# fxxJuses/MICFormer

Hardware: AMD Instinct MI355X
Metric: train volumes/sec (128^3 CT+MRI pair) (higher is better)
Workload: dtype bf16; 1 GPU; MicFormer base Head(embed_dim=48, depths 2-2-6-2, heads 3-6-12-24, window 2^3, 8 classes) full train step (fwd + MDiceLoss + bwd + Adam/cosine) on 128^3 CT+MR pairs, DropPath on; local_batch=2, global_batch=2, parallelism=dp1, launch=hipGraph replay (one graph)

## Files before the change

### micformer_amd/csrc/common.h

```cpp
#pragma once
#include <hip/hip_runtime.h>
#include <stdint.h>

#include "../../include/micformer_hip.h"
#include "gemm_core.h"

#define MICF_RETURN_LAUNCH()                          \
  do {                                                \
    return hipGetLastError() == hipSuccess ? MICF_OK : MICF_ELAUNCH; \
  } while (0)

namespace micf {

struct Options {
  int block_wave = 1;
  int block_recompute_h = 0;
  int block_debug = 0;
  int sample_tile = 1;
  int sample_e = -1;
  int cell_cap = -1;
  int tile_cap_hits = -1, tile_cap_cell = -1, tile_cap_voxel = -1;
};
Options& options();

struct Geo {
  int B, D, H, W;
  FastDiv fW, fH, fD;
  Geo() {}
  Geo(int B_, int D_, int H_, int W_) : B(B_), D(D_), H(H_), W(W_), fW((uint32_t)W_), fH((uint32_t)H_), fD((uint32_t)D_) {}
  __host__ __device__ int64_t tokens() const { return (int64_t)B * D * H * W; }
  __device__ __forceinline__ void decode(int t, int& b, int& d, int& h, int& w) const {
    uint32_t q, r;
    fW.divmod((uint32_t)t, q, r); w = (int)r;
    fH.divmod(q, q, r); h = (int)r;
    fD.divmod(q, q, r); d = (int)r; b = (int)q;
  }
  __device__ __forceinline__ int token(int b, int d, int h, int w) const { return ((b * D + d) * H + h) * W + w; }
};

__device__ __forceinline__ float wave_sum(float v) {
#pragma unroll
  for (int o = 32; o > 0; o >>= 1) v += __shfl_xor(v, o, 64);
  return v;
}

int colsum_atomic(const float* dy, const float* scale, int64_t rps, float* out, int64_t M, int N, hipStream_t s);

constexpr int kOffsetHidden = 16;
struct CellLists {
  int* count;
  int* ovf_count;
  int* list;
  int* ovf;
  int cap;
  float* w8;
};
struct SampleFwdSet { const float *h, *ln_g, *ln_b, *w1, *xa; float *flow, *xs; };
struct SampleBwdSet {
  const float *dxs, *h, *ln_g, *ln_b, *w1, *xa, *flow;
  float *dxa, *dh, *dln_g, *dln_b, *dw1;
  CellLists cl;
  float* partials;
};
int offset_sample_fwd_groups(const SampleFwdSet* sets, int n, int B, int D, int H, int W, int C, float eps, hipStream_t stream);
int offset_sample_bwd_groups(SampleBwdSet* sets, int n, int B, int D, int H, int W, int C, float eps, float* workspace,
                             int64_t workspace_floats, hipStream_t s, int phase = 0);
struct SampleFinishCall { const SampleBwdSet* sets; int n, B, D, H, W, C; float* workspace; int64_t workspace_floats; };
int offset_sample_finish_many(const SampleFinishCall* calls, int ncalls, hipStream_t s);

struct Conv3FwdSet { const float* x1; const float* x2; const float* w; const float* bias; float* y; float* wt; };
struct Conv3BwdSet { const float* dy; const float* w; float* wt; float* dx1; float* dx2; };
int conv3_fwd_x_groups(const Conv3FwdSet* sets, int n, int c1, int c2, int B, int D, int H, int W, int N, hipStream_t stream, int dtype,
                       int prepared, int y_zeroed);
bool conv3_fwd_x_splits(int B, int D, int H, int W, int c1, int c2);
int conv3_bwd_data_x_groups(const Conv3BwdSet* sets, int ng, int c1, int acc1, int c2, int acc2, int B, int D, int H, int W, int N,
                            hipStream_t stream, int dtype, int prepared);

int conv3_bwd_data_x(const float* dy, const float* w, float* wt, float* dx1, int c1, int acc1, float* dx2, int c2, int acc2, int B,
                     int D, int H, int W, int N, hipStream_t stream, int dtype = 0, int prepared = 0);

int64_t conv3_fwdx_workspace(int N, int c1, int c2);
int conv3_fwd_x(const float* x1, int c1, const float* x2, int c2, const float* w, const float* bias, float* y, float* wt, int B, int D,
                int H, int W, int N, hipStream_t stream, int dtype = 0, int prepared = 0);
int64_t conv3_wgradx_workspace(int B, int D, int H, int W, int N, int c1, int c2, int items = 1);
int conv3_wgradx_items(const float* const* dy, const float* const* x1, const float* const* x2, float* const* dw, float* const* dbias,
                       int n, int c1, int c2, int B, int D, int H, int W, int N, float* ws, int64_t ws_floats, hipStream_t stream,
                       int dtype);
int conv3_wgradx(const float* dy, const float* x1, int c1, const float* x2, int c2, float* dw, float* dbias, int B, int D, int H,
                 int W, int N, float* ws, int64_t ws_floats, hipStream_t stream, int dtype = 0);

}
```

### micformer_amd/csrc/conv3_bwdx.hip

```cpp
#include <cstdlib>
#include "common.h"
#include "conv3_layout.h"
#include "gemm_dma.h"

namespace micf {

constexpr int xKS = 20;

struct BwdxArgs {
  const float* dy; int N;
  const float* wt;
  float* d1; float* d2; int oc1, oc2, acc1, acc2;
  int O;
  int B, D, H, W, tiles_d, tiles_h, tiles_w, ngroups;
  const float* dyb; const float* wtb; float* d1b; float* d2b;
};

__global__ void __launch_bounds__(256) conv3_wt_kernel(const float* __restrict__ w, float* __restrict__ wt, int N, int Cin) {
  const int64_t id = (int64_t)blockIdx.x * 256 + threadIdx.x;
  if (id < conv3_bwd_layout_items(Cin)) conv3_bwd_layout_write(w, wt, N, Cin, id);
}

template <int TW, int NCT, bool BF16>
__global__ void __launch_bounds__(256) conv3_bwdx_kernel(BwdxArgs a) {
  constexpr int CH = 16 / TW, TH = 4 * CH, TD = 2;
  constexpr int HD = TD + 2, HH = TH + 2, HW = TW + 2, HALO = HD * HH * HW;
  __shared__ __attribute__((aligned(16))) float Xs[HALO * xKS];
  if (blockIdx.z) { a.dy = a.dyb; a.wt = a.wtb; a.d1 = a.d1b; a.d2 = a.d2b; }
  const int tid = threadIdx.x, lane = tid & 63, wave = __builtin_amdgcn_readfirstlane(tid >> 6), li = lane & 15, lr = lane >> 4;
  int q = blockIdx.x;
  if (gridDim.x >= 64 && (gridDim.x & 7) == 0) q = (q & 7) * (gridDim.x >> 3) + (q >> 3);
  const int tw = q % a.tiles_w; q /= a.tiles_w;
  const int th = q % a.tiles_h; q /= a.tiles_h;
  const int td = q % a.tiles_d; const int b = q / a.tiles_d;
  const int d0 = td * TD, h0 = th * TH, w0 = tw * TW;
  const int64_t DHW = (int64_t)a.D * a.H * a.W;
  const int ct0 = blockIdx.y * NCT;
  const int nct = min(NCT, a.O / 16 - ct0);

  {
    constexpr int NH = (HALO * 4 + 255) / 256;
    float4 hv4[NH];
#pragma unroll
    for (int it = 0; it < NH; ++it) {
      const int idx = tid + it * 256;
      hv4[it] = make_float4(0.f, 0.f, 0.f, 0.f);
      if (idx < HALO * 4) {
        const int hv = idx >> 2, g = idx & 3;
        const int hw = hv % HW, hh = (hv / HW) % HH, hd = hv / (HW * HH);
        const int dd = d0 + hd - 1, yy = h0 + hh - 1, ww = w0 + hw - 1;
        if ((unsigned)dd < (unsigned)a.D && (unsigned)yy < (unsigned)a.H && (unsigned)ww < (unsigned)a.W && 4 * g < a.N)
          hv4[it] = *reinterpret_cast<const float4*>(a.dy + ((int64_t)b * DHW + ((int64_t)dd * a.H + yy) * a.W + ww) * a.N + 4 * g);
      }
    }
#pragma unroll
    for (int it = 0; it < NH; ++it) {
      const int idx = tid + it * 256;
      if (idx < HALO * 4) {
        if constexpr (BF16)
          *reinterpret_cast<uint2*>(&reinterpret_cast<uint16_t*>(Xs)[(idx >> 2) * xKS + 4 * (idx & 3)]) =
              make_uint2(pack_bf16(hv4[it].x, hv4[it].y), pack_bf16(hv4[it].z, hv4[it].w));
        else
          *reinterpret_cast<float4*>(&Xs[(idx >> 2) * xKS + 4 * (idx & 3)]) = hv4[it];
      }
    }
  }
  int ld[2], lh[2], lw[2];
#pragma unroll
  for (int tj = 0; tj < 2; ++tj) {
    const int ct = 2 * wave + tj;
    ld[tj] = ct / 4;
    lh[tj] = (ct % 4) * CH + li / TW;
    lw[tj] = li % TW;
  }
  f32x4 acc[NCT][2];
#pragma unroll
  for (int t = 0; t < NCT; ++t) { acc[t][0] = f32x4{0.f, 0.f, 0.f, 0.f}; acc[t][1] = f32x4{0.f, 0.f, 0.f, 0.f}; }
  const float* wp = a.wt + ((int64_t)(ct0 * 16 + li)) * 16 + 4 * lr;
  const int64_t tap_stride = (int64_t)a.O * 16;
  if constexpr (BF16) {
    typedef unsigned u32x4 __attribute__((ext_vector_type(4)));
    const uint16_t* Xh = reinterpret_cast<const uint16_t*>(Xs);
    const u32x4* wq = reinterpret_cast<const u32x4*>(reinterpret_cast<const uint16_t*>(a.wt + conv3_bwd_layout_f32(a.O)) +
                                                     (((int64_t)(ct0 * 16 + li)) * 4 + lr) * 8);
    const int64_t pair_stride = (int64_t)a.O * 4;
// ... 64 lines not shown
  for (int t = 0; t < NCT; ++t) av[t] = (t < nct && !BF16) ? *reinterpret_cast<const float4*>(wp + t * 256) : make_float4(0.f, 0.f, 0.f, 0.f);
  if constexpr (!BF16) __syncthreads();
#pragma unroll 1
  for (int tap = 0; tap < (BF16 ? 0 : 27); ++tap) {
    if (tap + 1 < 27) {
#pragma unroll
      for (int t = 0; t < NCT; ++t)
        an[t] = (t < nct) ? *reinterpret_cast<const float4*>(wp + (tap + 1) * tap_stride + t * 256) : make_float4(0.f, 0.f, 0.f, 0.f);
    }
    const int kd = tap / 9, kh = (tap / 3) % 3, kw = tap % 3;
    float4 bv[2];
#pragma unroll
    for (int tj = 0; tj < 2; ++tj) {
      const int zd = ld[tj] + 2 - kd, zh = lh[tj] + 2 - kh, zw = lw[tj] + 2 - kw;
      bv[tj] = *reinterpret_cast<const float4*>(&Xs[((zd * HH + zh) * HW + zw) * xKS + 4 * lr]);
    }
    if constexpr (!BF16) {
#pragma unroll
      for (int s = 0; s < 4; ++s) {
        const float b0 = s == 0 ? bv[0].x : (s == 1 ? bv[0].y : (s == 2 ? bv[0].z : bv[0].w));
        const float b1 = s == 0 ? bv[1].x : (s == 1 ? bv[1].y : (s == 2 ? bv[1].z : bv[1].w));
#pragma unroll
        for (int t = 0; t < NCT; ++t) {
          const float av_s = s == 0 ? av[t].x : (s == 1 ? av[t].y : (s == 2 ? av[t].z : av[t].w));
          acc[t][0] = __builtin_amdgcn_mfma_f32_16x16x4f32(av_s, b0, acc[t][0], 0, 0, 0);
          acc[t][1] = __builtin_amdgcn_mfma_f32_16x16x4f32(av_s, b1, acc[t][1], 0, 0, 0);
        }
      }
    } else {
      if ((tap & 1) || tap == 26) {
        const float4 z = make_float4(0.f, 0.f, 0.f, 0.f);
        const bool pair = tap & 1;
        const bf16x8 bb0 = pair ? to_bf16x8(bprev[0], bv[0]) : to_bf16x8(bv[0], z);
        const bf16x8 bb1 = pair ? to_bf16x8(bprev[1], bv[1]) : to_bf16x8(bv[1], z);
#pragma unroll
        for (int t = 0; t < NCT; ++t) {
          const bf16x8 ba = pair ? to_bf16x8(aprev[t], av[t]) : to_bf16x8(av[t], z);
          acc[t][0] = __builtin_amdgcn_mfma_f32_16x16x32_bf16(ba, bb0, acc[t][0], 0, 0, 0);
          acc[t][1] = __builtin_amdgcn_mfma_f32_16x16x32_bf16(ba, bb1, acc[t][1], 0, 0, 0);
        }
      } else {
        bprev[0] = bv[0]; bprev[1] = bv[1];
#pragma unroll
        for (int t = 0; t < NCT; ++t) aprev[t] = av[t];
      }
    }
#pragma unroll
    for (int t = 0; t < NCT; ++t) av[t] = an[t];
  }
#pragma unroll
  for (int tj = 0; tj < 2; ++tj) {
    const int dd = d0 + ld[tj], yy = h0 + lh[tj], ww = w0 + lw[tj];
    if (dd >= a.D || yy >= a.H || ww >= a.W) continue;
    const int64_t tok = (int64_t)b * DHW + ((int64_t)dd * a.H + yy) * a.W + ww;
    auto where = [&](int t, int& accf) -> float* {
      const int c = (ct0 + t) * 16 + 4 * lr;
      if (t >= nct) return nullptr;
      if (c < a.oc1) { accf = a.acc1; return a.d1 ? a.d1 + tok * a.oc1 + c : nullptr; }
      accf = a.acc2;
      return a.d2 ? a.d2 + tok * a.oc2 + (c - a.oc1) : nullptr;
    };
    constexpr int EB = NCT >= 6 ? 2 : NCT;
#pragma unroll
    for (int t0 = 0; t0 < NCT; t0 += EB) {
      float4 old[EB];
#pragma unroll
      for (int u = 0; u < EB; ++u) {
        int accf = 0;
        const float* p = where(t0 + u, accf);
        old[u] = (p && accf) ? *reinterpret_cast<const float4*>(p) : make_float4(0.f, 0.f, 0.f, 0.f);
      }
#pragma unroll
      for (int u = 0; u < EB; ++u) {
        int accf = 0;
        float* p = where(t0 + u, accf);
        if (!p) continue;
        const f32x4 v = acc[t0 + u][tj];
        *reinterpret_cast<float4*>(p) = make_float4(v[0] + old[u].x, v[1] + old[u].y, v[2] + old[u].z, v[3] + old[u].w);
      }
    }
  }
}

template <int TW, bool BF16>
static hipError_t launch_bwdx(BwdxArgs& a, hipStream_t stream) {
  constexpr int CH = 16 / TW, TH = 4 * CH;
  a.tiles_d = (a.D + 1) / 2;
  a.tiles_h = (a.H + TH - 1) / TH;
  a.tiles_w = (a.W + TW - 1) / TW;
  const int64_t blocks = (int64_t)a.B * a.tiles_d * a.tiles_h * a.tiles_w;
  const int cts = a.O / 16;
  if (blocks * ((cts + 5) / 6) >= 128)
    hipLaunchKernelGGL((conv3_bwdx_kernel<TW, 6, BF16>), dim3((unsigned)blocks, (cts + 5) / 6, a.ngroups), dim3(256), 0, stream, a);
  else
    hipLaunchKernelGGL((conv3_bwdx_kernel<TW, 2, BF16>), dim3((unsigned)blocks, (cts + 1) / 2, a.ngroups), dim3(256), 0, stream, a);
  return hipGetLastError();
}

int conv3_bwd_data_x(const float* dy, const float* w, float* wt, float* dx1, int c1, int acc1, float* dx2, int c2, int acc2, int B,
                     int D, int H, int W, int N, hipStream_t stream, int dtype, int prepared) {
  const Conv3BwdSet one{dy, w, wt, dx1, dx2};
  return conv3_bwd_data_x_groups(&one, 1, c1, acc1, c2, acc2, B, D, H, W, N, stream, dtype, prepared);
}

int conv3_bwd_data_x_groups(const Conv3BwdSet* sets, int ng, int c1, int acc1, int c2, int acc2, int B, int D, int H, int W, int N,
                            hipStream_t stream, int dtype, int prepared) {
  if (!sets || ng < 1 || ng > 2) return MICF_EINVAL;
  const int O = c1 + c2;
  if (N > 16 || (N & 3) || (O & 15) || (c1 & 3) || (c2 & 3) || W < 4) return MICF_EUNSUPPORTED;
  for (int i = 0; i < ng; ++i)
    if (!aligned16(sets[i].dy) || !aligned16(sets[i].wt) || (sets[i].dx1 && !aligned16(sets[i].dx1)) || (sets[i].dx2 && !aligned16(sets[i].dx2)) ||
        (!sets[i].dx1) != (!sets[0].dx1) || (!sets[i].dx2) != (!sets[0].dx2))
      return MICF_EUNSUPPORTED;
  const float *dy = sets[0].dy;
  float *wt = sets[0].wt, *dx1 = sets[0].dx1, *dx2 = sets[0].dx2;
  const int64_t n = conv3_bwd_layout_items(O);
  if (!prepared) {
    for (int i = 0; i < ng; ++i) {
      hipLaunchKernelGGL(conv3_wt_kernel, dim3((unsigned)((n + 255) / 256)), dim3(256), 0, stream, sets[i].w, sets[i].wt, N, O);
      if (hipGetLastError() != hipSuccess) return MICF_ELAUNCH;
    }
  }
  BwdxArgs a{};
  a.dyb = sets[ng - 1].dy; a.wtb = sets[ng - 1].wt; a.d1b = sets[ng - 1].dx1; a.d2b = sets[ng - 1].dx2; a.ngroups = ng;
  a.dy = dy; a.N = N; a.wt = wt; a.d1 = dx1; a.d2 = dx2; a.oc1 = c1; a.oc2 = c2; a.acc1 = acc1; a.acc2 = acc2; a.O = O;
  a.B = B; a.D = D; a.H = H; a.W = W;
  const hipError_t e = dtype == MICF_DTYPE_BF16 ? ((W >= 12) ? launch_bwdx<16, true>(a, stream) : launch_bwdx<8, true>(a, stream))
                                                 : ((W >= 12) ? launch_bwdx<16, false>(a, stream) : launch_bwdx<8, false>(a, stream));
  return e == hipSuccess ? MICF_OK : MICF_ELAUNCH;
}

}
```

### micformer_amd/csrc/conv3_fwdx.hip

```cpp
#include <cstdlib>
#include "common.h"
#include "conv3_layout.h"
#include "gemm_dma.h"

namespace micf {

constexpr int fKS = 20;
constexpr int fAhead = 3;

struct FwdxArgs {
  const float* x1; const float* x2; int c1, c2;
  const float* wt;
  const float* bias; float* y; int N;
  const float* x1b; const float* x2b; const float* wtb; const float* biasb; float* yb;
  int B, D, H, W, tiles_d, tiles_h, tiles_w;
  int chunks, chunks_per_block;
};

__global__ void __launch_bounds__(256) conv3_wtf_kernel(const float* __restrict__ w, float* __restrict__ wt, int N, int Cin, int chunks) {
  const int64_t id = (int64_t)blockIdx.x * 256 + threadIdx.x;
  if (id < conv3_fwd_layout_items(Cin)) conv3_fwd_layout_write(w, wt, N, Cin, id);
}

template <int TW, bool BF16>
__global__ void __launch_bounds__(256) conv3_fwdx_kernel(FwdxArgs a) {
  constexpr int CH = 16 / TW, TH = 4 * CH, TD = 2;
  constexpr int HD = TD + 2, HH = TH + 2, HW = TW + 2, HALO = HD * HH * HW;
  constexpr int NH = (HALO * 4 + 255) / 256;
  __shared__ __attribute__((aligned(16))) float Xs[HALO * fKS];
  if (blockIdx.z) { a.x1 = a.x1b; a.x2 = a.x2b; a.wt = a.wtb; a.bias = a.biasb; a.y = a.yb; }
  const int tid = threadIdx.x, lane = tid & 63, wave = __builtin_amdgcn_readfirstlane(tid >> 6), li = lane & 15, lr = lane >> 4;
  int q = blockIdx.x;
  if (gridDim.x >= 64 && (gridDim.x & 7) == 0) q = (q & 7) * (gridDim.x >> 3) + (q >> 3);
  const int tw = q % a.tiles_w; q /= a.tiles_w;
  const int th = q % a.tiles_h; q /= a.tiles_h;
  const int td = q % a.tiles_d; const int b = q / a.tiles_d;
  const int d0 = td * TD, h0 = th * TH, w0 = tw * TW;
  const int64_t DHW = (int64_t)a.D * a.H * a.W;
  const int Cin = a.c1 + a.c2;
  const int kc_begin = blockIdx.y * a.chunks_per_block;
  const int kc_end = min(a.chunks, kc_begin + a.chunks_per_block);

  auto fetch = [&](int kc, float4 (&hv)[NH]) {
#pragma unroll
    for (int it = 0; it < NH; ++it) {
      const int idx = tid + it * 256;
      hv[it] = make_float4(0.f, 0.f, 0.f, 0.f);
      if (idx < HALO * 4) {
        const int v = idx >> 2, g = idx & 3;
        const int hw = v % HW, hh = (v / HW) % HH, hd = v / (HW * HH);
        const int dd = d0 + hd - 1, yy = h0 + hh - 1, ww = w0 + hw - 1;
        const int c = kc * 16 + 4 * g;
        if ((unsigned)dd < (unsigned)a.D && (unsigned)yy < (unsigned)a.H && (unsigned)ww < (unsigned)a.W && c < Cin) {
          const int64_t tok = (int64_t)b * DHW + ((int64_t)dd * a.H + yy) * a.W + ww;
          hv[it] = c < a.c1 ? *reinterpret_cast<const float4*>(a.x1 + tok * a.c1 + c)
                            : *reinterpret_cast<const float4*>(a.x2 + tok * a.c2 + (c - a.c1));
        }
      }
    }
  };
  uint16_t* Xh = reinterpret_cast<uint16_t*>(Xs);
  auto commit = [&](const float4 (&hv)[NH]) {
#pragma unroll
    for (int it = 0; it < NH; ++it) {
      const int idx = tid + it * 256;
      if (idx < HALO * 4) {
        if constexpr (BF16)
          *reinterpret_cast<uint2*>(&Xh[(idx >> 2) * fKS + 4 * (idx & 3)]) = make_uint2(pack_bf16(hv[it].x, hv[it].y), pack_bf16(hv[it].z, hv[it].w));
        else
          *reinterpret_cast<float4*>(&Xs[(idx >> 2) * fKS + 4 * (idx & 3)]) = hv[it];
      }
    }
  };

  int vbase[2];
#pragma unroll
  for (int tj = 0; tj < 2; ++tj) {
    const int ct = 2 * wave + tj;
    const int ld = ct / 4, lh = (ct % 4) * CH + li / TW, lw = li % TW;
    vbase[tj] = ((ld * HH + lh) * HW + lw) * fKS + 4 * lr;
  }
  f32x4 acc[2] = {f32x4{0.f, 0.f, 0.f, 0.f}, f32x4{0.f, 0.f, 0.f, 0.f}};
  float4 hv[NH];
  fetch(kc_begin, hv);
  for (int kc = kc_begin; kc < kc_end; ++kc) {
// ... 17 lines not shown
#pragma unroll
        for (int e = 0; e < 2; ++e) {
          const int tap = 2 * p + e;
          if (tap < 27) {
            const int kd = tap / 9, kh = (tap / 3) % 3, kw = tap % 3;
            const int off = ((kd * HH + kh) * HW + kw) * fKS;
            h[e][0] = *reinterpret_cast<const uint2*>(&Xh[vbase[0] + off]);
            h[e][1] = *reinterpret_cast<const uint2*>(&Xh[vbase[1] + off]);
          } else {
            h[e][0] = make_uint2(0u, 0u); h[e][1] = h[e][0];
          }
        }
        const u32x4 q0 = {h[0][0].x, h[0][0].y, h[1][0].x, h[1][0].y}, q1 = {h[0][1].x, h[0][1].y, h[1][1].x, h[1][1].y};
        acc[0] = __builtin_amdgcn_mfma_f32_16x16x32_bf16(__builtin_bit_cast(bf16x8, aq), __builtin_bit_cast(bf16x8, q0), acc[0], 0, 0, 0);
        acc[1] = __builtin_amdgcn_mfma_f32_16x16x32_bf16(__builtin_bit_cast(bf16x8, aq), __builtin_bit_cast(bf16x8, q1), acc[1], 0, 0, 0);
      }
      continue;
    }
    float4 ring[fAhead + 1];
    float4 aprev = make_float4(0.f, 0.f, 0.f, 0.f);
    uint2 hprev0 = make_uint2(0u, 0u), hprev1 = hprev0;
#pragma unroll
    for (int t = 0; t < fAhead; ++t) ring[t] = *reinterpret_cast<const float4*>(wp + t * 256);
#pragma unroll
    for (int tap = 0; tap < 27; ++tap) {
      if (tap + fAhead < 27) ring[(tap + fAhead) % (fAhead + 1)] = *reinterpret_cast<const float4*>(wp + (tap + fAhead) * 256);
      const float4 av = ring[tap % (fAhead + 1)];
      const int kd = tap / 9, kh = (tap / 3) % 3, kw = tap % 3;
      const int off = ((kd * HH + kh) * HW + kw) * fKS;
      if constexpr (!BF16) {
        const float4 b0 = *reinterpret_cast<const float4*>(&Xs[vbase[0] + off]);
        const float4 b1 = *reinterpret_cast<const float4*>(&Xs[vbase[1] + off]);
        acc[0] = __builtin_amdgcn_mfma_f32_16x16x4f32(av.x, b0.x, acc[0], 0, 0, 0);
        acc[1] = __builtin_amdgcn_mfma_f32_16x16x4f32(av.x, b1.x, acc[1], 0, 0, 0);
        acc[0] = __builtin_amdgcn_mfma_f32_16x16x4f32(av.y, b0.y, acc[0], 0, 0, 0);
        acc[1] = __builtin_amdgcn_mfma_f32_16x16x4f32(av.y, b1.y, acc[1], 0, 0, 0);
        acc[0] = __builtin_amdgcn_mfma_f32_16x16x4f32(av.z, b0.z, acc[0], 0, 0, 0);
        acc[1] = __builtin_amdgcn_mfma_f32_16x16x4f32(av.z, b1.z, acc[1], 0, 0, 0);
        acc[0] = __builtin_amdgcn_mfma_f32_16x16x4f32(av.w, b0.w, acc[0], 0, 0, 0);
        acc[1] = __builtin_amdgcn_mfma_f32_16x16x4f32(av.w, b1.w, acc[1], 0, 0, 0);
      } else {
        typedef unsigned u32x4 __attribute__((ext_vector_type(4)));
        const uint2 h0 = *reinterpret_cast<const uint2*>(&Xh[vbase[0] + off]);
        const uint2 h1 = *reinterpret_cast<const uint2*>(&Xh[vbase[1] + off]);
        if ((tap & 1) || tap == 26) {
          const float4 z = make_float4(0.f, 0.f, 0.f, 0.f);
          const bool pair = tap & 1;
          const bf16x8 ba = pair ? to_bf16x8(aprev, av) : to_bf16x8(av, z);
          const u32x4 q0 = pair ? u32x4{hprev0.x, hprev0.y, h0.x, h0.y} : u32x4{h0.x, h0.y, 0u, 0u};
          const u32x4 q1 = pair ? u32x4{hprev1.x, hprev1.y, h1.x, h1.y} : u32x4{h1.x, h1.y, 0u, 0u};
          acc[0] = __builtin_amdgcn_mfma_f32_16x16x32_bf16(ba, __builtin_bit_cast(bf16x8, q0), acc[0], 0, 0, 0);
          acc[1] = __builtin_amdgcn_mfma_f32_16x16x32_bf16(ba, __builtin_bit_cast(bf16x8, q1), acc[1], 0, 0, 0);
        } else {
          aprev = av; hprev0 = h0; hprev1 = h1;
        }
      }
    }
  }
  const bool atomic_out = gridDim.y > 1;
  const int n0 = 4 * lr;
#pragma unroll
  for (int tj = 0; tj < 2; ++tj) {
    const int ct = 2 * wave + tj;
    const int dd = d0 + ct / 4, yy = h0 + (ct % 4) * CH + li / TW, ww = w0 + li % TW;
    if (dd >= a.D || yy >= a.H || ww >= a.W || n0 >= a.N) continue;
    float* p = a.y + ((int64_t)b * DHW + ((int64_t)dd * a.H + yy) * a.W + ww) * a.N + n0;
    f32x4 v = acc[tj];
    if (a.bias && blockIdx.y == 0) {
#pragma unroll
      for (int e = 0; e < 4; ++e) if (n0 + e < a.N) v[e] += a.bias[n0 + e];
    }
    if (atomic_out) {
#pragma unroll
      for (int e = 0; e < 4; ++e) if (n0 + e < a.N) atomicAdd(p + e, v[e]);
    } else if (n0 + 3 < a.N && (a.N & 3) == 0) {
      *reinterpret_cast<float4*>(p) = make_float4(v[0], v[1], v[2], v[3]);
    } else {
#pragma unroll
      for (int e = 0; e < 4; ++e) if (n0 + e < a.N) p[e] = v[e];
    }
  }
}

int64_t conv3_fwdx_workspace(int N, int c1, int c2) {
  if (N <= 0 || N > 16 || c1 + c2 <= 0) return 0;
  return conv3_fwd_layout_floats(c1 + c2);
}

int conv3_fwd_x(const float* x1, int c1, const float* x2, int c2, const float* w, const float* bias, float* y, float* wt, int B, int D,
                int H, int W, int N, hipStream_t stream, int dtype, int prepared) {
  const Conv3FwdSet one{x1, x2, w, bias, y, wt};
  return conv3_fwd_x_groups(&one, 1, c1, c2, B, D, H, W, N, stream, dtype, prepared, 0);
}

bool conv3_fwd_x_splits(int B, int D, int H, int W, int c1, int c2) {
  const int chunks = (c1 + c2 + 15) / 16;
  const int tw_ = W >= 12 ? 16 : 8, th_ = 4 * (16 / tw_);
  const int64_t blocks = (int64_t)B * ((D + 1) / 2) * ((H + th_ - 1) / th_) * ((W + tw_ - 1) / tw_);
  return blocks < 256 && chunks > 1;
}

int conv3_fwd_x_groups(const Conv3FwdSet* sets, int n, int c1, int c2, int B, int D, int H, int W, int N, hipStream_t stream, int dtype,
                       int prepared, int y_zeroed) {
  if (!sets || n < 1 || n > 2) return MICF_EINVAL;
  if (N > 16 || (c1 & 3) || (c2 & 3) || W < 4) return MICF_EUNSUPPORTED;
  for (int i = 0; i < n; ++i)
    if (!aligned16(sets[i].x1) || (sets[i].x2 && !aligned16(sets[i].x2)) || !aligned16(sets[i].y) || !aligned16(sets[i].wt)) return MICF_EUNSUPPORTED;
  const float *x1 = sets[0].x1, *x2 = sets[0].x2, *w = sets[0].w, *bias = sets[0].bias;
  float *y = sets[0].y, *wt = sets[0].wt;
  const int Cin = c1 + c2, chunks = (Cin + 15) / 16;
  const int64_t nw = conv3_fwd_layout_items(Cin);
  if (!prepared) {
    for (int i = 0; i < n; ++i) {
      hipLaunchKernelGGL(conv3_wtf_kernel, dim3((unsigned)((nw + 255) / 256)), dim3(256), 0, stream, sets[i].w, sets[i].wt, N, Cin, chunks);
      if (hipGetLastError() != hipSuccess) return MICF_ELAUNCH;
    }
  }
  FwdxArgs a{};
  a.x1 = x1; a.x2 = x2 ? x2 : x1; a.c1 = c1; a.c2 = c2; a.wt = wt; a.bias = bias; a.y = y; a.N = N;
  a.B = B; a.D = D; a.H = H; a.W = W; a.chunks = chunks;
  const Conv3FwdSet& sb = sets[n - 1];
  a.x1b = sb.x1; a.x2b = sb.x2 ? sb.x2 : sb.x1; a.wtb = sb.wt; a.biasb = sb.bias; a.yb = sb.y;
  const int tw_ = W >= 12 ? 16 : 8, th_ = 4 * (16 / tw_);
  a.tiles_d = (D + 1) / 2; a.tiles_h = (H + th_ - 1) / th_; a.tiles_w = (W + tw_ - 1) / tw_;
  const int64_t blocks = (int64_t)B * a.tiles_d * a.tiles_h * a.tiles_w;
  int ysplit = 1;
  constexpr int split_target = 128;
  if (blocks < 256) { ysplit = (int)((split_target + blocks - 1) / blocks); if (ysplit > chunks) ysplit = chunks; if (ysplit < 1) ysplit = 1; }
  a.chunks_per_block = (chunks + ysplit - 1) / ysplit;
  ysplit = (chunks + a.chunks_per_block - 1) / a.chunks_per_block;
  if (ysplit > 1 && !y_zeroed)
    for (int i = 0; i < n; ++i)
      if (hipMemsetAsync(sets[i].y, 0, sizeof(float) * (size_t)B * D * H * W * N, stream) != hipSuccess) return MICF_ELAUNCH;
  const dim3 grid((unsigned)blocks, ysplit, n);
  if (dtype == MICF_DTYPE_BF16) {
    if (tw_ == 16) hipLaunchKernelGGL((conv3_fwdx_kernel<16, true>), grid, dim3(256), 0, stream, a);
    else hipLaunchKernelGGL((conv3_fwdx_kernel<8, true>), grid, dim3(256), 0, stream, a);
  } else {
    if (tw_ == 16) hipLaunchKernelGGL((conv3_fwdx_kernel<16, false>), grid, dim3(256), 0, stream, a);
    else hipLaunchKernelGGL((conv3_fwdx_kernel<8, false>), grid, dim3(256), 0, stream, a);
  }
  return hipGetLastError() == hipSuccess ? MICF_OK : MICF_ELAUNCH;
}

}
```

### micformer_amd/csrc/misc.hip

```cpp
#include <hip/hip_fp16.h>

#include "common.h"
#include <string.h>

namespace micf {

__global__ void __launch_bounds__(256) pad3d_kernel(const float* __restrict__ src, float* __restrict__ dst, int B, int D, int H,
                                                    int W, int Dp, int Hp, int Wp, int C, int64_t total) {
  for (int64_t i = (int64_t)blockIdx.x * 256 + threadIdx.x; i < total; i += (int64_t)gridDim.x * 256) {
    int64_t t = i / C; const int c = (int)(i - t * C);
    const int w = (int)(t % Wp); t /= Wp; const int h = (int)(t % Hp); t /= Hp; const int d = (int)(t % Dp); const int b = (int)(t / Dp);
    dst[i] = (d < D && h < H && w < W) ? src[((((int64_t)b * D + d) * H + h) * W + w) * C + c] : 0.f;
  }
}
__global__ void __launch_bounds__(256) crop3d_kernel(const float* __restrict__ src, float* __restrict__ dst, int B, int D, int H,
                                                     int W, int Dp, int Hp, int Wp, int C, int accumulate, int64_t total) {
  for (int64_t i = (int64_t)blockIdx.x * 256 + threadIdx.x; i < total; i += (int64_t)gridDim.x * 256) {
    int64_t t = i / C; const int c = (int)(i - t * C);
    const int w = (int)(t % W); t /= W; const int h = (int)(t % H); t /= H; const int d = (int)(t % D); const int b = (int)(t / D);
    const float v = src[((((int64_t)b * Dp + d) * Hp + h) * Wp + w) * C + c];
    dst[i] = accumulate ? dst[i] + v : v;
  }
}

__device__ __forceinline__ void ac_coord(int o, int Sin, int Sout, int& i0, int& i1, float& f) {
  const float scale = Sout > 1 ? (float)(Sin - 1) / (float)(Sout - 1) : 0.f;
  const float s = scale * (float)o;
  i0 = (int)s; if (i0 > Sin - 1) i0 = Sin - 1;
  i1 = i0 + (i0 < Sin - 1 ? 1 : 0);
  f = s - (float)i0;
}
template <bool BWD>
__global__ void __launch_bounds__(256) resize_kernel(const float* __restrict__ a, float* __restrict__ o, int B, int D, int H, int W,
                                                     int Do, int Ho, int Wo, int C, int64_t total) {
  for (int64_t i = (int64_t)blockIdx.x * 256 + threadIdx.x; i < total; i += (int64_t)gridDim.x * 256) {
    int64_t t = i / C; const int c = (int)(i - t * C);
    const int w = (int)(t % Wo); t /= Wo; const int h = (int)(t % Ho); t /= Ho; const int d = (int)(t % Do); const int b = (int)(t / Do);
    int d0, d1, h0, h1, w0, w1; float fd, fh, fw;
    ac_coord(d, D, Do, d0, d1, fd); ac_coord(h, H, Ho, h0, h1, fh); ac_coord(w, W, Wo, w0, w1, fw);
    float acc = 0.f;
    const float gv = BWD ? a[i] : 0.f;
#pragma unroll
    for (int q = 0; q < 8; ++q) {
      const int dd = (q & 4) ? d1 : d0, hh = (q & 2) ? h1 : h0, ww = (q & 1) ? w1 : w0;
      const float wt = ((q & 4) ? fd : 1.f - fd) * ((q & 2) ? fh : 1.f - fh) * ((q & 1) ? fw : 1.f - fw);
      const int64_t s = ((((int64_t)b * D + dd) * H + hh) * W + ww) * C + c;
      if (BWD) atomicAdd(o + s, wt * gv); else acc += wt * a[s];
    }
    if (!BWD) o[i] = acc;
  }
}

}
using namespace micf;

extern "C" int micf_abi_version(void) { return MICF_ABI_VERSION; }

micf::Options& micf::options() {
  static Options o;
  return o;
}

static int* option_slot(const char* name) {
  if (!name) return nullptr;
  Options& o = micf::options();
  const struct { const char* n; int* v; } table[] = {
      {"block_wave", &o.block_wave}, {"block_recompute_h", &o.block_recompute_h}, {"block_debug", &o.block_debug},
      {"sample_tile", &o.sample_tile}, {"sample_e", &o.sample_e}, {"cell_cap", &o.cell_cap},
      {"tile_cap_hits", &o.tile_cap_hits}, {"tile_cap_cell", &o.tile_cap_cell}, {"tile_cap_voxel", &o.tile_cap_voxel}};
  for (const auto& e : table)
    if (!strcmp(name, e.n)) return e.v;
  return nullptr;
}

extern "C" int micf_set_option(const char* name, int value) {
  int* slot = option_slot(name);
  if (!slot) return MICF_EINVAL;
  *slot = value;
  return MICF_OK;
}

extern "C" int micf_get_option(const char* name, int* value) {
  const int* slot = option_slot(name);
  if (!slot || !value) return MICF_EINVAL;
  *value = *slot;
  return MICF_OK;
}

extern "C" const char* micf_strerror(int code) {
  switch (code) {
    case MICF_OK: return "ok";
    case MICF_EINVAL: return "invalid argument (null pointer, bad size or misaligned buffer)";
    case MICF_EUNSUPPORTED: return "shape not supported by the HIP kernels";
    case MICF_ELAUNCH: return "HIP kernel launch failed";
    default: return "unknown micf error code";
  }
}

static int grid_for(int64_t total) { int64_t b = (total + 255) / 256; return (int)(b > 16384 ? 16384 : (b < 1 ? 1 : b)); }

extern "C" int micf_pad3d(const float* src, float* dst, int B, int D, int H, int W, int Dp, int Hp, int Wp, int C,
                          micf_stream_t stream) {
  if (!src || !dst || B <= 0 || D <= 0 || H <= 0 || W <= 0 || C <= 0 || Dp < D || Hp < H || Wp < W) return MICF_EINVAL;
  const int64_t total = (int64_t)B * Dp * Hp * Wp * C;
  hipLaunchKernelGGL(pad3d_kernel, dim3(grid_for(total)), dim3(256), 0, (hipStream_t)stream, src, dst, B, D, H, W, Dp, Hp, Wp, C, total);
  MICF_RETURN_LAUNCH();
}
extern "C" int micf_crop3d(const float* src, float* dst, int B, int D, int H, int W, int Dp, int Hp, int Wp, int C, int accumulate,
                           micf_stream_t stream) {
  if (!src || !dst || B <= 0 || D <= 0 || H <= 0 || W <= 0 || C <= 0 || Dp < D || Hp < H || Wp < W) return MICF_EINVAL;
  const int64_t total = (int64_t)B * D * H * W * C;
  hipLaunchKernelGGL(crop3d_kernel, dim3(grid_for(total)), dim3(256), 0, (hipStream_t)stream, src, dst, B, D, H, W, Dp, Hp, Wp, C,
                     accumulate, total);
  MICF_RETURN_LAUNCH();
}
extern "C" int micf_resize_trilinear_fwd(const float* src, float* dst, int B, int D, int H, int W, int Do, int Ho, int Wo, int C,
                                         micf_stream_t stream) {
  if (!src || !dst || B <= 0 || D <= 0 || H <= 0 || W <= 0 || Do <= 0 || Ho <= 0 || Wo <= 0 || C <= 0) return MICF_EINVAL;
  const int64_t total = (int64_t)B * Do * Ho * Wo * C;
  hipLaunchKernelGGL(resize_kernel<false>, dim3(grid_for(total)), dim3(256), 0, (hipStream_t)stream, src, dst, B, D, H, W, Do, Ho, Wo, C, total);
  MICF_RETURN_LAUNCH();
}
extern "C" int micf_resize_trilinear_bwd(const float* ddst, float* dsrc, int B, int D, int H, int W, int Do, int Ho, int Wo, int C,
                                         micf_stream_t stream) {
  if (!ddst || !dsrc || B <= 0 || D <= 0 || H <= 0 || W <= 0 || Do <= 0 || Ho <= 0 || Wo <= 0 || C <= 0) return MICF_EINVAL;
  hipStream_t s = (hipStream_t)stream;
  if (hipMemsetAsync(dsrc, 0, sizeof(float) * (size_t)B * D * H * W * C, s) != hipSuccess) return MICF_ELAUNCH;
  const int64_t total = (int64_t)B * Do * Ho * Wo * C;
  hipLaunchKernelGGL(resize_kernel<true>, dim3(grid_for(total)), dim3(256), 0, s, ddst, dsrc, B, D, H, W, Do, Ho, Wo, C, total);
  MICF_RETURN_LAUNCH();
}

extern "C" int micf_zero(void* p, int64_t bytes, micf_stream_t stream) {
  if (!p || bytes < 0) return MICF_EINVAL;
  if (bytes == 0) return MICF_OK;
  return hipMemsetAsync(p, 0, (size_t)bytes, (hipStream_t)stream) == hipSuccess ? MICF_OK : MICF_ELAUNCH;
}

namespace micf {
__device__ __forceinline__ uint64_t mix64(uint64_t z) {
  z += 0x9E3779B97F4A7C15ull;
  z = (z ^ (z >> 30)) * 0xBF58476D1CE4E5B9ull;
  z = (z ^ (z >> 27)) * 0x94D049BB133111EBull;
  return z ^ (z >> 31);
}
__global__ void __launch_bounds__(256) drop_path_draw_kernel(uint64_t* __restrict__ rng, const float* __restrict__ keep,
                                                             float* __restrict__ out, int n, int B) {
  const uint64_t seed = rng[0], ctr = rng[1];
  for (int e = threadIdx.x; e < n * B; e += 256) {
    const float k = keep[e / B];
    const uint64_t h = mix64(mix64(seed ^ mix64(ctr)) + (uint64_t)e);
// ... 240 lines not shown
```

Baseline: 246.7 pairs/s.

## Add depth-marching 3D conv kernels with LDS-resident weights and plane ring buffer

Adds new forward and backward-data 3x3x3 conv kernels that keep one 96-channel weight set resident in LDS and march along depth. Input planes are held in a ring buffer, with the next plane prefetched into registers while MFMA runs on the current one. Each input plane is loaded once per depth range instead of being reloaded per tile, and the work splits over depth ranges with an XCD-aware block order. The new path is on by default for bf16 with channels divisible by 96. In exchange it uses up to 160KB of dynamic LDS, and the forward pass with multiple channel sets needs atomic output and a memset.

```diff
diff --git a/micformer_amd/csrc/common.h b/micformer_amd/csrc/common.h
--- a/micformer_amd/csrc/common.h
+++ b/micformer_amd/csrc/common.h
@@ -19,6 +19,7 @@
   int sample_tile = 1;
   int sample_e = -1;
   int cell_cap = -1;
+  int conv_march = 1;
   int tile_cap_hits = -1, tile_cap_cell = -1, tile_cap_voxel = -1;
 };
 Options& options();
diff --git a/micformer_amd/csrc/conv3_bwdx.hip b/micformer_amd/csrc/conv3_bwdx.hip
--- a/micformer_amd/csrc/conv3_bwdx.hip
+++ b/micformer_amd/csrc/conv3_bwdx.hip
@@ -1,6 +1,7 @@
 #include <cstdlib>
 #include "common.h"
 #include "conv3_layout.h"
+#include "conv3_march_plan.h"
 #include "gemm_dma.h"
 
 namespace micf {
@@ -231,6 +232,171 @@
   }
 }
 
+struct BwdmArgs {
+  BwdxArgs x;
+  micf_march::Plan plan;
+};
+
+__global__ void __launch_bounds__(256) conv3_bwdm_kernel(BwdmArgs m) {
+  namespace P = micf_march;
+  typedef unsigned u32x4 __attribute__((ext_vector_type(4)));
+  constexpr int HH = 10, HW = P::kHaloW, PV = HH * HW;
+  constexpr int NV = (PV * 4 + 255) / 256;
+  constexpr int NCT = 6, WQ = P::kWeightBytes / 16;
+  static_assert(P::kBwdVoxelBytes == 2 * xKS && P::kBwdRing == 4 && WQ % 256 == 0, "LDS carve-up");
+  extern __shared__ __attribute__((aligned(16))) char bwdm_smem[];
+  u32x4* Wl = reinterpret_cast<u32x4*>(bwdm_smem);
+  uint16_t* Xh = reinterpret_cast<uint16_t*>(bwdm_smem + P::kWeightBytes);
+  BwdxArgs& a = m.x;
+  if (blockIdx.z) { a.dy = a.dyb; a.wt = a.wtb; a.d1 = a.d1b; a.d2 = a.d2b; }
+  const int tid = threadIdx.x, lane = tid & 63, wave = __builtin_amdgcn_readfirstlane(tid >> 6), li = lane & 15, lr = lane >> 4;
+  const P::Unit u = P::decode(m.plan, blockIdx.x);
+  const int ct0 = blockIdx.y * NCT;
+  const int64_t DHW = (int64_t)a.D * a.H * a.W;
+
+  auto fetch = [&](int plane, float4 (&hv)[NV], bool (&keep)[NV]) {
+    const bool zp = P::zero_plane(m.plan, plane);
+    const int pc = min(max(plane, 0), a.D - 1);
+#pragma unroll
+    for (int it = 0; it < NV; ++it) {
+      const int idx = min(tid + it * 256, PV * 4 - 1);
+      const int v = idx >> 2, g = idx & 3;
+      const int yy = u.h0 + v / HW - 1, ww = u.w0 + v % HW - 1;
+      const bool in = !zp && (unsigned)yy < (unsigned)a.H && (unsigned)ww < (unsigned)a.W;
+      const int64_t tok = (int64_t)u.b * DHW + ((int64_t)pc * a.H + min(max(yy, 0), a.H - 1)) * a.W + min(max(ww, 0), a.W - 1);
+      hv[it] = *reinterpret_cast<const float4*>(a.dy + tok * 16 + 4 * g);
+      keep[it] = in;
+    }
+  };
+  auto commit = [&](int plane, float4 (&hv)[NV], const bool (&keep)[NV]) {
+#pragma unroll
+    for (int it = 0; it < NV; ++it) {
+      asm volatile("" : "+v"(hv[it].x), "+v"(hv[it].y), "+v"(hv[it].z), "+v"(hv[it].w));
+      if (!keep[it]) hv[it] = make_float4(0.f, 0.f, 0.f, 0.f);
+    }
+    uint16_t* dst = Xh + ((plane + 1) & 3) * (PV * xKS);
+#pragma unroll
+    for (int it = 0; it < NV; ++it) {
+      const int idx = tid + it * 256;
+      if (idx < PV * 4)
+        *reinterpret_cast<uint2*>(&dst[(idx >> 2) * xKS + 4 * (idx & 3)]) = make_uint2(pack_bf16(hv[it].x, hv[it].y), pack_bf16(hv[it].z, hv[it].w));
+    }
+  };
+
+  {
+    const u32x4* wq = reinterpret_cast<const u32x4*>(reinterpret_cast<const uint16_t*>(a.wt + conv3_bwd_layout_f32(a.O))) + ct0 * 64;
+    const int64_t pair_stride = (int64_t)a.O * 4;
+    constexpr int WB = WQ / 256;
+    u32x4 r[WB];
+    float4 h0v[NV], h1v[NV], h2v[NV];
+    bool k0[NV], k1[NV], k2[NV];
+    fetch(u.d0 - 1, h0v, k0); fetch(u.d0, h1v, k1); fetch(u.d0 + 1, h2v, k2);
+#pragma unroll
+    for (int k = 0; k < WB; ++k) {
+      const int idx = tid + k * 256;
+      r[k] = wq[(idx / (NCT * 64)) * pair_stride + idx % (NCT * 64)];
+    }
+    __builtin_amdgcn_sched_barrier(0);
+    commit(u.d0 - 1, h0v, k0); commit(u.d0, h1v, k1); commit(u.d0 + 1, h2v, k2);
+#pragma unroll
+    for (int k = 0; k < WB; ++k) Wl[tid + k * 256] = r[k];
+  }
+  __syncthreads();
+
+  const int hh0 = u.h0 + 2 * wave, ww = u.w0 + li;
+  const int vb = ((2 * wave + 2) * HW + li + 2) * xKS + 4 * lr;
+  const u32x4* wl = Wl + li * 4 + lr;
+
+#pragma unroll 1
+  for (int d = u.d0; d < u.d1; ++d) {
+    float4 hv[NV];
+    bool hk[NV];
+    const bool more = d + 2 <= u.d1;
+    if (more) fetch(d + 2, hv, hk);
+    float* op[2][NCT];
+    float4 old[2][NCT];
+#pragma unroll
+    for (int tj = 0; tj < 2; ++tj) {
+      const bool tokv = hh0 + tj < a.H && ww < a.W;
+      const int64_t tok = (int64_t)u.b * DHW + ((int64_t)d * a.H + hh0 + tj) * a.W + ww;
+#pragma unroll
+      for (int t = 0; t < NCT; ++t) {
+        const int c = (ct0 + t) * 16 + 4 * lr;
+        float* p;
+        int accf;
+        if (c < a.oc1) { accf = a.acc1; p = a.d1 ? a.d1 + tok * a.oc1 + c : nullptr; }
+        else { accf = a.acc2; p = a.d2 ? a.d2 + tok * a.oc2 + (c - a.oc1) : nullptr; }
+        if (!tokv) p = nullptr;
+        op[tj][t] = p;
+        old[tj][t] = (p && accf) ? *reinterpret_cast<const float4*>(p) : make_float4(0.f, 0.f, 0.f, 0.f);
+      }
+    }
+    f32x4 acc[NCT][2];
+#pragma unroll
+    for (int t = 0; t < NCT; ++t) { acc[t][0] = f32x4{0.f, 0.f, 0.f, 0.f}; acc[t][1] = f32x4{0.f, 0.f, 0.f, 0.f}; }
+    int sb[3];
+#pragma unroll
+    for (int kd = 0; kd < 3; ++kd) sb[kd] = ((d + 2 - kd) & 3) * (PV * xKS) + vb;
+    u32x4 fa[2][NCT];
+    uint2 fh[2][2][2];
+    auto request = [&](int p, u32x4 (&qa)[NCT], uint2 (&qh)[2][2]) {
+#pragma unroll
+      for (int t = 0; t < NCT; ++t) qa[t] = wl[(p * P::kSetChannels + t * 16) * 4];
+#pragma unroll
+      for (int tj = 0; tj < 2; ++tj)
+#pragma unroll
+        for (int e = 0; e < 2; ++e) {
+          const int tap = 2 * p + e;
+          if (tap < 27) {
+            const int kd = tap / 9, kh = (tap / 3) % 3, kw = tap % 3;
+            qh[tj][e] = *reinterpret_cast<const uint2*>(&Xh[sb[kd] + ((tj - kh) * HW - kw) * xKS]);
+          } else {
+            qh[tj][e] = make_uint2(0u, 0u);
+          }
+        }
+    };
+    request(0, fa[0], fh[0]);
+#pragma unroll
+    for (int p = 0; p < P::kPairs; ++p) {
+      if (p + 1 < P::kPairs) request(p + 1, fa[(p + 1) & 1], fh[(p + 1) & 1]);
+      __builtin_amdgcn_sched_barrier(0);
+      u32x4 bq[2];
+#pragma unroll
+      for (int tj = 0; tj < 2; ++tj) bq[tj] = u32x4{fh[p & 1][tj][0].x, fh[p & 1][tj][0].y, fh[p & 1][tj][1].x, fh[p & 1][tj][1].y};
+#pragma unroll
+      for (int t = 0; t < NCT; ++t) {
+        acc[t][0] = __builtin_amdgcn_mfma_f32_16x16x32_bf16(__builtin_bit_cast(bf16x8, fa[p & 1][t]), __builtin_bit_cast(bf16x8, bq[0]), acc[t][0], 0, 0, 0);
+        acc[t][1] = __builtin_amdgcn_mfma_f32_16x16x32_bf16(__builtin_bit_cast(bf16x8, fa[p & 1][t]), __builtin_bit_cast(bf16x8, bq[1]), acc[t][1], 0, 0, 0);
+      }
+      __builtin_amdgcn_sched_barrier(0);
+    }
+    if (more) commit(d + 2, hv, hk);
+#pragma unroll
+    for (int tj = 0; tj < 2; ++tj)
+#pragma unroll
+      for (int t = 0; t < NCT; ++t) {
+        if (!op[tj][t]) continue;
+        const f32x4 v = acc[t][tj];
+        const float4 o = old[tj][t];
+        *reinterpret_cast<float4*>(op[tj][t]) = make_float4(v[0] + o.x, v[1] + o.y, v[2] + o.z, v[3] + o.w);
+      }
+    __syncthreads();
+  }
+}
+
+static hipError_t launch_bwdm(const BwdxArgs& a, const micf_march::Plan& plan, hipStream_t stream) {
+  namespace P = micf_march;
+  static bool attr_set = false;
+  if (!attr_set) {
+    if (hipFuncSetAttribute(reinterpret_cast<const void*>(&conv3_bwdm_kernel), hipFuncAttributeMaxDynamicSharedMemorySize, P::kLdsLimit) != hipSuccess)
+      return hipErrorInvalidValue;
+    attr_set = true;
+  }
+  BwdmArgs m{a, plan};
+  hipLaunchKernelGGL(conv3_bwdm_kernel, dim3((unsigned)plan.parts, plan.sets, plan.groups), dim3(256), (size_t)P::lds_bytes(plan), stream, m);
+  return hipGetLastError();
+}
+
 template <int TW, bool BF16>
 static hipError_t launch_bwdx(BwdxArgs& a, hipStream_t stream) {
   constexpr int CH = 16 / TW, TH = 4 * CH;
@@ -274,6 +440,11 @@
   a.dyb = sets[ng - 1].dy; a.wtb = sets[ng - 1].wt; a.d1b = sets[ng - 1].dx1; a.d2b = sets[ng - 1].dx2; a.ngroups = ng;
   a.dy = dy; a.N = N; a.wt = wt; a.d1 = dx1; a.d2 = dx2; a.oc1 = c1; a.oc2 = c2; a.acc1 = acc1; a.acc2 = acc2; a.O = O;
   a.B = B; a.D = D; a.H = H; a.W = W;
+  const int march = options().conv_march;
+  if (march && dtype == MICF_DTYPE_BF16 && N == 16 && micf_march::supported(micf_march::kBwd, W, O)) {
+    const micf_march::Plan plan = micf_march::make_plan(micf_march::kBwd, B, D, H, W, O, ng);
+    if (march == 2 || micf_march::fills_chip(plan)) return launch_bwdm(a, plan, stream) == hipSuccess ? MICF_OK : MICF_ELAUNCH;
+  }
   const hipError_t e = dtype == MICF_DTYPE_BF16 ? ((W >= 12) ? launch_bwdx<16, true>(a, stream) : launch_bwdx<8, true>(a, stream))
                                                  : ((W >= 12) ? launch_bwdx<16, false>(a, stream) : launch_bwdx<8, false>(a, stream));
   return e == hipSuccess ? MICF_OK : MICF_ELAUNCH;
diff --git a/micformer_amd/csrc/conv3_fwdx.hip b/micformer_amd/csrc/conv3_fwdx.hip
--- a/micformer_amd/csrc/conv3_fwdx.hip
+++ b/micformer_amd/csrc/conv3_fwdx.hip
@@ -1,6 +1,7 @@
 #include <cstdlib>
 #include "common.h"
 #include "conv3_layout.h"
+#include "conv3_march_plan.h"
 #include "gemm_dma.h"
 
 namespace micf {
@@ -184,6 +185,167 @@
   }
 }
 
+struct FwdmArgs {
+  FwdxArgs x;
+  micf_march::Plan plan;
+};
+
+__global__ void __launch_bounds__(256) conv3_fwdm_kernel(FwdmArgs m) {
+  namespace P = micf_march;
+  typedef unsigned u32x4 __attribute__((ext_vector_type(4)));
+  constexpr int HH = 6, HW = P::kHaloW, PV = HH * HW;
+  constexpr int VS = P::kFwdVoxelBytes / 2;
+  constexpr int NG = P::kSetChannels / 4;
+  constexpr int NV = (PV * NG + 255) / 256;
+  constexpr int WQ = P::kWeightBytes / 16;
+  static_assert(P::kFwdRing == 3 && WQ % 256 == 0 && P::kFwdVoxelBytes % 8 == 0, "LDS carve-up");
+  extern __shared__ __attribute__((aligned(16))) char fwdm_smem[];
+  u32x4* Wl = reinterpret_cast<u32x4*>(fwdm_smem);
+  uint16_t* Xh = reinterpret_cast<uint16_t*>(fwdm_smem + P::kWeightBytes);
+  FwdxArgs& a = m.x;
+  if (blockIdx.z) { a.x1 = a.x1b; a.x2 = a.x2b; a.wt = a.wtb; a.bias = a.biasb; a.y = a.yb; }
+  const int tid = threadIdx.x, lane = tid & 63, wave = __builtin_amdgcn_readfirstlane(tid >> 6), li = lane & 15, lr = lane >> 4;
+  const P::Unit u = P::decode(m.plan, blockIdx.x);
+  const int64_t DHW = (int64_t)a.D * a.H * a.W;
+  const int set = blockIdx.y, c0 = set * P::kSetChannels;
+
+  auto fetch = [&](int plane, float4 (&hv)[NV], bool (&keep)[NV]) {
+    const bool zp = P::zero_plane(m.plan, plane);
+    const int pc = min(max(plane, 0), a.D - 1);
+#pragma unroll
+    for (int it = 0; it < NV; ++it) {
+      const int idx = min(tid + it * 256, PV * NG - 1);
+      const int v = idx / NG, c = c0 + 4 * (idx % NG);
+      const int yy = u.h0 + v / HW - 1, ww = u.w0 + v % HW - 1;
+      const bool in = !zp && (unsigned)yy < (unsigned)a.H && (unsigned)ww < (unsigned)a.W;
+      const int64_t tok = (int64_t)u.b * DHW + ((int64_t)pc * a.H + min(max(yy, 0), a.H - 1)) * a.W + min(max(ww, 0), a.W - 1);
+      const float* src = c < a.c1 ? a.x1 + tok * a.c1 + c : a.x2 + tok * a.c2 + (c - a.c1);
+      hv[it] = *reinterpret_cast<const float4*>(src);
+      keep[it] = in;
+    }
+  };
+  auto commit = [&](int plane, float4 (&hv)[NV], const bool (&keep)[NV]) {
+#pragma unroll
+    for (int it = 0; it < NV; ++it) {
+      asm volatile("" : "+v"(hv[it].x), "+v"(hv[it].y), "+v"(hv[it].z), "+v"(hv[it].w));
+      if (!keep[it]) hv[it] = make_float4(0.f, 0.f, 0.f, 0.f);
+    }
+    uint16_t* dst = Xh + ((plane + 1) % 3) * (PV * VS);
+#pragma unroll
+    for (int it = 0; it < NV; ++it) {
+      const int idx = tid + it * 256;
+      if (idx < PV * NG)
+        *reinterpret_cast<uint2*>(&dst[(idx / NG) * VS + 4 * (idx % NG)]) = make_uint2(pack_bf16(hv[it].x, hv[it].y), pack_bf16(hv[it].z, hv[it].w));
+    }
+  };
+
+  {
+    const u32x4* wq = reinterpret_cast<const u32x4*>(reinterpret_cast<const uint16_t*>(a.wt + conv3_fwd_layout_f32(a.c1 + a.c2))) + set * WQ;
+    constexpr int WB = WQ / 256;
+    u32x4 r[WB];
+    float4 h0v[NV], h1v[NV];
+    bool k0[NV], k1[NV];
+    fetch(u.d0 - 1, h0v, k0);
+#pragma unroll
+    for (int k = 0; k < WB; ++k) r[k] = wq[tid + k * 256];
+    __builtin_amdgcn_sched_barrier(0);
+    commit(u.d0 - 1, h0v, k0);
+#pragma unroll
+    for (int k = 0; k < WB; ++k) Wl[tid + k * 256] = r[k];
+    __builtin_amdgcn_sched_barrier(0);
+    fetch(u.d0, h0v, k0); fetch(u.d0 + 1, h1v, k1);
+    __builtin_amdgcn_sched_barrier(0);
+    commit(u.d0, h0v, k0); commit(u.d0 + 1, h1v, k1);
+  }
+  __syncthreads();
+
+  const int hh = u.h0 + wave, ww = u.w0 + li;
+  const int vb = (wave * HW + li) * VS + 4 * lr;
+  const u32x4* wl = Wl + li * 4 + lr;
+  const bool tokv = hh < a.H && ww < a.W;
+  f32x4 bias4 = {0.f, 0.f, 0.f, 0.f};
+  const bool add_bias = a.bias && set == 0, atomic_out = gridDim.y > 1;
+  if (add_bias) {
+#pragma unroll
+    for (int e = 0; e < 4; ++e) bias4[e] = a.bias[4 * lr + e];
+  }
+
+#pragma unroll 1
+  for (int d = u.d0; d < u.d1; ++d) {
+    float4 hv[NV];
+    bool hk[NV];
+    const bool more = d + 2 <= u.d1;
+    if (more) fetch(d + 2, hv, hk);
+    int sb[3];
+#pragma unroll
+    for (int kd = 0; kd < 3; ++kd) sb[kd] = ((d + kd) % 3) * (PV * VS) + vb;
+    f32x4 acc = {0.f, 0.f, 0.f, 0.f};
+    constexpr int SP = P::kPairs / 2, NS = 2 * (P::kSetChannels / 16);
+    u32x4 fa[2][SP];
+    uint2 fh[2][2 * SP];
+    auto request = [&](int st, u32x4 (&qa)[SP], uint2 (&qh)[2 * SP]) {
+      const int kc = st >> 1, p0 = (st & 1) * SP;
+#pragma unroll
+      for (int j = 0; j < SP; ++j) qa[j] = wl[(kc * P::kPairs + p0 + j) * 64];
+#pragma unroll
+      for (int e = 0; e < 2 * SP; ++e) {
+        const int tap = 2 * p0 + e;
+        if (tap < 27) {
+          const int kd = tap / 9, kh = (tap / 3) % 3, kw = tap % 3;
+          qh[e] = *reinterpret_cast<const uint2*>(&Xh[sb[kd] + (kh * HW + kw) * VS + kc * 16]);
+        } else {
+          qh[e] = make_uint2(0u, 0u);
+        }
+      }
+    };
+    request(0, fa[0], fh[0]);
+#pragma unroll
+    for (int st = 0; st < NS; ++st) {
+      if (st + 1 < NS) request(st + 1, fa[(st + 1) & 1], fh[(st + 1) & 1]);
+      __builtin_amdgcn_sched_barrier(0);
+#pragma unroll
+      for (int j = 0; j < SP; ++j) {
+        const uint2 h0 = fh[st & 1][2 * j], h1 = fh[st & 1][2 * j + 1];
+        const u32x4 bq = {h0.x, h0.y, h1.x, h1.y};
+        acc = __builtin_amdgcn_mfma_f32_16x16x32_bf16(__builtin_bit_cast(bf16x8, fa[st & 1][j]), __builtin_bit_cast(bf16x8, bq), acc, 0, 0, 0);
+      }
+      __builtin_amdgcn_sched_barrier(0);
+    }
+    if (more) {
+      __syncthreads();
+      commit(d + 2, hv, hk);
+    }
+    if (tokv) {
+      float* p = a.y + ((int64_t)u.b * DHW + ((int64_t)d * a.H + hh) * a.W + ww) * 16 + 4 * lr;
+      f32x4 v = acc;
+      if (add_bias) {
+#pragma unroll
+        for (int e = 0; e < 4; ++e) v[e] += bias4[e];
+      }
+      if (atomic_out) {
+#pragma unroll
+        for (int e = 0; e < 4; ++e) atomicAdd(p + e, v[e]);
+      } else {
+        *reinterpret_cast<float4*>(p) = make_float4(v[0], v[1], v[2], v[3]);
+      }
+    }
+    if (more) __syncthreads();
+  }
+}
+
+static hipError_t launch_fwdm(const FwdxArgs& a, const micf_march::Plan& plan, hipStream_t stream) {
+  namespace P = micf_march;
+  static bool attr_set = false;
+  if (!attr_set) {
+    if (hipFuncSetAttribute(reinterpret_cast<const void*>(&conv3_fwdm_kernel), hipFuncAttributeMaxDynamicSharedMemorySize, P::kLdsLimit) != hipSuccess)
+      return hipErrorInvalidValue;
+    attr_set = true;
+  }
+  FwdmArgs m{a, plan};
+  hipLaunchKernelGGL(conv3_fwdm_kernel, dim3((unsigned)plan.parts, plan.sets, plan.groups), dim3(256), (size_t)P::lds_bytes(plan), stream, m);
+  return hipGetLastError();
+}
+
 int64_t conv3_fwdx_workspace(int N, int c1, int c2) {
   if (N <= 0 || N > 16 || c1 + c2 <= 0) return 0;
   return conv3_fwd_layout_floats(c1 + c2);
@@ -196,6 +358,7 @@
 }
 
 bool conv3_fwd_x_splits(int B, int D, int H, int W, int c1, int c2) {
+  if (options().conv_march && micf_march::supported(micf_march::kFwd, W, c1 + c2) && (c1 + c2) / micf_march::kSetChannels > 1) return true;
   const int chunks = (c1 + c2 + 15) / 16;
   const int tw_ = W >= 12 ? 16 : 8, th_ = 4 * (16 / tw_);
   const int64_t blocks = (int64_t)B * ((D + 1) / 2) * ((H + th_ - 1) / th_) * ((W + tw_ - 1) / tw_);
@@ -223,6 +386,16 @@
   a.B = B; a.D = D; a.H = H; a.W = W; a.chunks = chunks;
   const Conv3FwdSet& sb = sets[n - 1];
   a.x1b = sb.x1; a.x2b = sb.x2 ? sb.x2 : sb.x1; a.wtb = sb.wt; a.biasb = sb.bias; a.yb = sb.y;
+  const int march = options().conv_march;
+  if (march && dtype == MICF_DTYPE_BF16 && N == 16 && micf_march::supported(micf_march::kFwd, W, Cin)) {
+    const micf_march::Plan plan = micf_march::make_plan(micf_march::kFwd, B, D, H, W, Cin, n);
+    if (march == 2 || (micf_march::fills_chip(plan) && plan.sets > 1)) {
+      if (plan.sets > 1 && !y_zeroed)
+        for (int i = 0; i < n; ++i)
+          if (hipMemsetAsync(sets[i].y, 0, sizeof(float) * (size_t)B * D * H * W * N, stream) != hipSuccess) return MICF_ELAUNCH;
+      return launch_fwdm(a, plan, stream) == hipSuccess ? MICF_OK : MICF_ELAUNCH;
+    }
+  }
   const int tw_ = W >= 12 ? 16 : 8, th_ = 4 * (16 / tw_);
   a.tiles_d = (D + 1) / 2; a.tiles_h = (H + th_ - 1) / th_; a.tiles_w = (W + tw_ - 1) / tw_;
   const int64_t blocks = (int64_t)B * a.tiles_d * a.tiles_h * a.tiles_w;
diff --git a/micformer_amd/csrc/conv3_march_plan.h b/micformer_amd/csrc/conv3_march_plan.h
--- /dev/null
+++ b/micformer_amd/csrc/conv3_march_plan.h
@@ -0,0 +1,89 @@
+#pragma once
+#include <stdint.h>
+
+#if defined(__HIPCC__) || defined(__CUDACC__)
+#define MICF_MARCH_HD __host__ __device__ inline
+#else
+#define MICF_MARCH_HD inline
+#endif
+
+namespace micf_march {
+
+constexpr int kFwd = 0, kBwd = 1;
+constexpr int kSetChannels = 96;
+constexpr int kPairs = 14;
+constexpr int kWeightBytes = kPairs * kSetChannels * 64;
+constexpr int kTw = 16;
+constexpr int kHaloW = kTw + 2;
+constexpr int kWgTarget = 256;
+constexpr int kFillMin = 128;
+constexpr int kMinRange = 2;
+constexpr int kLdsLimit = 160 * 1024;
+constexpr int kBwdVoxelBytes = 40, kFwdVoxelBytes = 200;
+constexpr int kBwdRing = 4, kFwdRing = 3;
+
+struct Plan {
+  int form, B, D, H, W, channels, groups;
+  int th, tiles_h, tiles_w;
+  int sets;
+  int nranges;
+  int parts;
+  int xcd_order;
+};
+
+struct Unit { int b, h0, w0, d0, d1; };
+
+MICF_MARCH_HD bool supported(int form, int W, int channels) {
+  if (W < 12 || channels <= 0 || channels % kSetChannels) return false;
+  return form == kBwd || channels / kSetChannels <= 2;
+}
+
+MICF_MARCH_HD Plan make_plan(int form, int B, int D, int H, int W, int channels, int groups) {
+  Plan p;
+  p.form = form; p.B = B; p.D = D; p.H = H; p.W = W; p.channels = channels; p.groups = groups;
+  p.th = form == kBwd ? 8 : 4;
+  p.tiles_h = (H + p.th - 1) / p.th;
+  p.tiles_w = (W + kTw - 1) / kTw;
+  p.sets = channels / kSetChannels;
+  const int64_t units = (int64_t)groups * p.sets * B * p.tiles_h * p.tiles_w;
+  const int64_t want = (kWgTarget + units - 1) / units;
+  const int most = D / kMinRange > 1 ? D / kMinRange : 1;
+  p.nranges = (int)(want < most ? want : most);
+  p.parts = B * p.tiles_h * p.tiles_w * p.nranges;
+  p.xcd_order = p.parts % 8 == 0 ? 1 : 0;
+  return p;
+}
+
+MICF_MARCH_HD bool fills_chip(const Plan& p) { return (int64_t)p.parts * p.sets * p.groups >= kFillMin; }
+
+MICF_MARCH_HD int range_begin(const Plan& p, int r) { return (int)((int64_t)r * p.D / p.nranges); }
+
+MICF_MARCH_HD Unit decode(const Plan& p, int lin) {
+  int q = p.xcd_order ? (lin % 8) * (p.parts / 8) + lin / 8 : lin;
+  Unit u;
+  const int r = q % p.nranges; q /= p.nranges;
+  u.w0 = (q % p.tiles_w) * kTw; q /= p.tiles_w;
+  u.h0 = (q % p.tiles_h) * p.th;
+  u.b = q / p.tiles_h;
+  u.d0 = range_begin(p, r);
+  u.d1 = range_begin(p, r + 1);
+  return u;
+}
+
+MICF_MARCH_HD bool zero_plane(const Plan& p, int d) { return d < 0 || d >= p.D; }
+
+MICF_MARCH_HD int slots(const Plan& p) { return p.th * kTw; }
+
+MICF_MARCH_HD int64_t slot_token(const Plan& p, const Unit& u, int d, int slot) {
+  const int h = u.h0 + slot / kTw, w = u.w0 + slot % kTw;
+  if (h >= p.H || w >= p.W) return -1;
+  return (((int64_t)u.b * p.D + d) * p.H + h) * p.W + w;
+}
+
+MICF_MARCH_HD int plane_voxels(const Plan& p) { return (p.th + 2) * kHaloW; }
+MICF_MARCH_HD int plane_bytes(const Plan& p) { return plane_voxels(p) * (p.form == kBwd ? kBwdVoxelBytes : kFwdVoxelBytes); }
+MICF_MARCH_HD int ring_planes(const Plan& p) { return p.form == kBwd ? kBwdRing : kFwdRing; }
+MICF_MARCH_HD int ring_offset(const Plan&) { return kWeightBytes; }
+MICF_MARCH_HD int lds_bytes(const Plan& p) { return kWeightBytes + ring_planes(p) * plane_bytes(p); }
+
+}
diff --git a/micformer_amd/csrc/misc.hip b/micformer_amd/csrc/misc.hip
--- a/micformer_amd/csrc/misc.hip
+++ b/micformer_amd/csrc/misc.hip
@@ -66,7 +66,7 @@
   Options& o = micf::options();
   const struct { const char* n; int* v; } table[] = {
       {"block_wave", &o.block_wave}, {"block_recompute_h", &o.block_recompute_h}, {"block_debug", &o.block_debug},
-      {"sample_tile", &o.sample_tile}, {"sample_e", &o.sample_e}, {"cell_cap", &o.cell_cap},
+      {"sample_tile", &o.sample_tile}, {"sample_e", &o.sample_e}, {"cell_cap", &o.cell_cap}, {"conv_march", &o.conv_march},
       {"tile_cap_hits", &o.tile_cap_hits}, {"tile_cap_cell", &o.tile_cap_cell}, {"tile_cap_voxel", &o.tile_cap_voxel}};
   for (const auto& e : table)
     if (!strcmp(name, e.n)) return e.v;
```

Result: no change. 246.4 pairs/s (median of 2 runs) (-0.1%).
